# Gallicchio-Lab/openmm_agbnp_plugin

Measured on AMD Instinct MI355X. Metric: AGBNP1 force-eval-limited ns/day (1 fs step), thrombin 1dwc, independent replicas, higher is better.
Workload: dtype f64

## Files before the change

### openmm_agbnp_plugin_amd/csrc/agbnp_common.h

```cpp
#pragma once
#include <cfloat>
#include <cmath>
#include <cstddef>
#include <cstdint>

#ifdef __HIPCC__
#define AGBNP_HD __host__ __device__ __attribute__((always_inline))
#else
#define AGBNP_HD
#endif

namespace agbnp {

constexpr double kKFC = (2.2269859253f);
constexpr double kMinGvol = FLT_MIN;
constexpr int kMaxOrder = 8;
constexpr double kVolMinA = (0.01f * (0.001f));
constexpr double kVolMinB = (0.1f * (0.001f));
constexpr double kRadiusIncrement = (0.5f * (0.1f));
constexpr double kHBRadius = (1.4 * (0.1f));
constexpr double kSolventRadius = (1.0 * (0.1f));
constexpr double kI4MaxA = 2.0;
constexpr int kI4Nodes = 16;
constexpr int kLutStride = kI4Nodes + 1;
constexpr long kRadiusPrecision = 10000;
constexpr double kPi = 3.14159265358979323846;

constexpr double kToKjMol = 4.184 * 332.0 / 10.0;
constexpr double kDielFactor = kToKjMol * (-0.5) * (1. / 1.0 - 1. / 80.0);

struct SubtreeHeader {
  int nnodes;
  int natoms;
  int nroots;
  int npairs;
  int partners[8];
};



constexpr int kMaxItems = 8;
constexpr int kRowStride = 16;
AGBNP_HD constexpr size_t slot_row_item(size_t slot, size_t k) { return (size_t)kRowStride * slot + k; }
AGBNP_HD constexpr size_t slot_row_count(size_t slot) { return (size_t)kRowStride * slot + kMaxItems; }

constexpr int kWorkItemPartShift = 24, kWorkItemPartsShift = 26;
AGBNP_HD constexpr int make_work_item(int root, int part, int parts) {
  return root | (part << kWorkItemPartShift) | ((parts - 1) << kWorkItemPartsShift);
}
AGBNP_HD constexpr int work_item_root(int e) { return e & ((1 << kWorkItemPartShift) - 1); }
AGBNP_HD constexpr int work_item_part(int e) { return (e >> kWorkItemPartShift) & 3; }
AGBNP_HD constexpr int work_item_parts(int e) { return ((e >> kWorkItemPartsShift) & 3) + 1; }

constexpr int kTileBlocksMax = 4095;
constexpr int kTileStripFlag = 1 << 24;
AGBNP_HD constexpr int make_tile_item(int I, int J, int flag = 0) { return I | (J << 12) | flag; }
AGBNP_HD constexpr int tile_I(int item) { return item & 0xfff; }
AGBNP_HD constexpr int tile_J(int item) { return (item >> 12) & 0xfff; }

constexpr int kRowEntryTypeShift = 24;
AGBNP_HD constexpr unsigned make_row_entry(unsigned index, unsigned type) { return index | (type << kRowEntryTypeShift); }
AGBNP_HD constexpr unsigned row_entry_index(unsigned e) { return e & ((1u << kRowEntryTypeShift) - 1); }
AGBNP_HD constexpr unsigned row_entry_type(unsigned e) { return e >> kRowEntryTypeShift; }
constexpr int kRowItemSliceShift = 24;
AGBNP_HD constexpr unsigned make_row_item(unsigned list, unsigned slice) { return list | (slice << kRowItemSliceShift); }
AGBNP_HD constexpr unsigned row_item_list(unsigned it) { return it & ((1u << kRowItemSliceShift) - 1); }
AGBNP_HD constexpr unsigned row_item_slice(unsigned it) { return it >> kRowItemSliceShift; }

enum PackingWord {
  kPackForestsNext = 1,
  kPackForestsNow = 2,
  kPackState = 3,
};
enum PackStateWord {
  kPsLevel = 0,
  kPsAge = 1,
  kPsClean = 2,
  kPsPlans = 3,
  kPsTotalNodes = 4,
  kPsMaxNodes = 5,
  kPsEpoch = 6,
  kPsHeat = 7,
  kPsNeed = 8,
  kPsWords = 9,
  kPsReported = kPsPlans + 1
};
constexpr size_t packing_words(size_t slot_cap) { return slot_cap + kPackState + kPsWords; }

enum RowFlagWord {
  kNlStale = 0,
// ... 55 lines not shown
```

### openmm_agbnp_plugin_amd/csrc/engine_setup.hip

```cpp
#include "engine_context.h"

thread_local std::string g_create_error;

EngineSettings read_settings() {
  EngineSettings s;
  if (const char* v = getenv("AGBNP_HIP_FIVE_LAUNCHES")) s.five_launches = atoi(v) != 0;
  if (const char* v = getenv("AGBNP_HIP_ROWS")) s.rows = atoi(v) != 0 ? 1 : 0;
  if (const char* v = getenv("AGBNP_HIP_HEAL")) s.heal = atoi(v) != 0;
  if (const char* v = getenv("AGBNP_HIP_SPLIT_FIT")) s.split_fit = atoi(v) != 0;
  if (const char* v = getenv("AGBNP_HIP_GB_FAR")) s.gb_far = atoi(v) != 0 ? 1 : 0;
  if (const char* v = getenv("AGBNP_HIP_ROUND_PERMILLE")) s.round_permille = std::max(100, atoi(v));
  if (const char* v = getenv("AGBNP_HIP_REPLAN_EVERY")) s.replan_every = std::max(1, atoi(v));
  if (const char* v = getenv("AGBNP_HIP_ADAPTER_LAUNCH")) s.adapter_launch = atoi(v) != 0;
  if (getenv("AGBNP_HIP_NO_PINNED_STAGING")) s.pinned_staging = false;
  if (const char* v = getenv("AGBNP_HIP_SKIN")) s.skin = std::min(1.0, std::max(0.0, atof(v)));
  if (const char* v = getenv("AGBNP_HIP_ROW_MOVE")) s.row_move = std::max(atof(v), 0.0);
  if (const char* v = getenv("AGBNP_HIP_ROW_SLICE")) s.row_slice = atoi(v);
  if (const char* v = getenv("AGBNP_HIP_ROW_FILL")) s.row_fill = std::max(0.01, atof(v));
  if (const char* v = getenv("AGBNP_HIP_ROW_STRIDE")) s.row_stride = std::max(128, atoi(v));
  if (const char* v = getenv("AGBNP_HIP_MASK_SKIN")) s.mask_skin = std::min(0.5, std::max(0.0, atof(v)));
  if (const char* v = getenv("AGBNP_HIP_GROUP_LAUNCHES")) s.group_launches = atoi(v) != 0;
  return s;
}

// ... 180 lines not shown
  P.tree_atom_cap = tree_variant_atom_cap(c->variant);
  P.pack_enabled = 1;
  c->T.want_sv_large = c->diagnostics ? 1 : 0;
  apply_parity(c);
}

int mark_rows_stale(agbnp_hip_context* c) {
  const int stale = 1;
  HIP_TRY(c, hipMemcpy(c->d_nl_flag.p + kNlStale, &stale, sizeof(int), hipMemcpyHostToDevice));
  return AGBNP_HIP_OK;
}

namespace {

int allocate_rows(agbnp_hip_context* c) {
  const int n = c->n, nh = c->nh;
  PairArgs& P = c->P;
  constexpr int kRowCap = 3072;
  constexpr int kMaxTypes = 255;
  constexpr size_t kMaxTableBytes = 40 * 1024;
  constexpr int kMaxParticles = 65536;
  if (c->version != 1 || nh == 0 || n > kMaxParticles || c->cfg.rows == 0) return AGBNP_HIP_OK;
  if (c->lut.nscreened > kMaxTypes || c->lut.nscreener > kMaxTypes) return AGBNP_HIP_OK;
  if ((size_t)c->lut.nscreened * c->lut.nscreener * (kI4Nodes - 1) * 2 * sizeof(double2) > kMaxTableBytes) return AGBNP_HIP_OK;
  c->skin = c->cfg.skin;
  c->row_move = c->cfg.row_move;
  c->row_slice = c->cfg.row_slice;
  auto sorted_by_type = [&](int count, auto type_of) {
    std::vector<unsigned> v;
    for (int k = 0; k < count; k++) v.push_back(make_row_entry((unsigned)k, (unsigned)type_of(k)));
    std::stable_sort(v.begin(), v.end(), [](unsigned a, unsigned b) { return row_entry_type(a) < row_entry_type(b); });
    while (v.size() % 64 != 0) v.push_back(~0u);
    return v;
  };
  const std::vector<unsigned> hperm = sorted_by_type(nh, [&](int h) { return c->lut.type_screener[c->h2a[h]]; });
  const std::vector<unsigned> aperm = sorted_by_type(n, [&](int a) { return c->lut.type_screened[a]; });
  HIP_TRY(c, device_array(c, &P.hperm, hperm));
  HIP_TRY(c, device_array(c, &P.aperm, aperm));
  P.hperm_n = (int)hperm.size();
  P.aperm_n = (int)aperm.size();
  auto part_stride = [&](size_t candidates, int parts) { return std::max(128, std::min(64 * (int)((candidates / 64 + parts - 1) / parts), kRowCap)); };
  static_assert(kRowCap % 256 == 0, "a list is walked in slices of 256 entries");
  P.nlh_stride = part_stride(hperm.size(), kBornParts);
  P.nla_stride = part_stride(aperm.size(), kChainParts);
  {
    const double r = c->cutoff + c->skin + 0.3;
    const double most = 2.0 * 105.0 * (4.0 / 3.0) * M_PI * r * r * r / kGbParts;
    P.nlg_stride = c->method != 0 && c->cutoff > 0.0 && c->cutoff < 3.0
                       ? std::max(256, std::min(part_stride(aperm.size(), kGbParts), (int)((most + 255) / 256) * 256)) : 0;
  }
  if (c->cfg.row_stride > 0) {
    P.nlh_stride = P.nla_stride = c->cfg.row_stride;
    if (P.nlg_stride) P.nlg_stride = P.nlh_stride;
  }
  const size_t born_lists = (size_t)row_groups(n) * kBornParts, chain_lists = (size_t)row_groups(nh) * kChainParts;
  const size_t gb_lists = P.nlg_stride > 0 ? (size_t)row_groups(n) * kGbParts : 0;
  HIP_TRY(c, device_array(c, &P.nlh, born_lists * P.nlh_stride, 0));
  HIP_TRY(c, device_array(c, &P.nla, chain_lists * P.nla_stride, 0));
  HIP_TRY(c, device_array(c, &P.nlh_count, born_lists, 0));
  HIP_TRY(c, device_array(c, &P.nla_count, chain_lists, 0));
  {
    std::vector<unsigned> bs(row_groups(n), 0u), cs(row_groups(nh), 0u);
    for (int a = 0; a < n; a++) bs[a / kRowGroup] |= (unsigned)c->lut.type_screened[a] << (8 * (a % kRowGroup));
    for (int h = 0; h < nh; h++) cs[h / kRowGroup] |= (unsigned)c->lut.type_screener[c->h2a[h]] << (8 * (h % kRowGroup));
    HIP_TRY(c, device_array(c, &P.bslice, bs));
    HIP_TRY(c, device_array(c, &P.cslice, cs));
  }
  if (gb_lists > 0) {
    HIP_TRY(c, device_array(c, &P.nlg, gb_lists * P.nlg_stride, 0));
    HIP_TRY(c, device_array(c, &P.nlg_count, gb_lists, 0));
    const size_t waves = (gb_lists + 7) / 8 * 8 * (size_t)((P.nlg_stride + 255) / 256);
    HIP_TRY(c, c->d_egb_rows.alloc(waves, 0));
  }
  {
    const size_t most = std::max(std::max(born_lists * ((P.nlh_stride + 255) / 256), chain_lists * ((P.nla_stride + 255) / 256)),
                                 gb_lists * ((P.nlg_stride + 255) / 256));
    P.nl_items_cap = (int)std::min<size_t>(most + 8, 1u << 30);
    HIP_TRY(c, device_array(c, &P.nl_items, (size_t)kRowKinds * kRowBuffers * P.nl_items_cap, 0));
    HIP_TRY(c, device_array(c, &P.nl_nitems, kRowKinds * kRowBuffers, 0));
  }
  std::vector<int> flag(kNlFlagWords, 0);
  flag[kNlStale] = 1;
  flag[kNlSlice] = c->row_slice > 0 ? std::min(std::max(c->row_slice, kRowSlice), kRowSliceMax) / 64 * 64 : kRowSlice;
  HIP_TRY(c, c->d_nl_flag.upload(flag));
  P.nl_flag = c->d_nl_flag.p;
  HIP_TRY(c, device_array(c, &P.nl_ref, 3 * (size_t)n, 0xff));
  HIP_TRY(c, device_array(c, &P.bw, n, 0));
  HIP_TRY(c, device_array(c, &P.rec_h, nh));
  HIP_TRY(c, device_array(c, &P.hrow, nh));
  HIP_TRY(c, device_array(c, &P.grec, n, 0));
  HIP_TRY(c, device_array(c, &P.hrec, nh, 0));
  const int nti = c->lut.nscreened, ntj = c->lut.nscreener, ni = kI4Nodes - 1;
  const size_t tab = (size_t)nti * ntj * ni;
  const double dr = kI4MaxA / (kI4Nodes - 1);
  std::vector<double2> pw(4 * tab);
  for (int ti = 0; ti < nti; ti++)
    for (int tj = 0; tj < ntj; tj++)
      for (int k = 0; k < ni; k++) {
        const size_t o = ((size_t)ti * ntj + tj) * kI4Nodes + k;
        const double y0 = c->lut.y[o], y1 = c->lut.y[o + 1], z0 = c->lut.y2[o] * dr * dr / 6.0, z1 = c->lut.y2[o + 1] * dr * dr / 6.0;
        const double2 ca = make_double2(y0, (y1 - y0) - std::fma(2.0, z0, z1)), cb = make_double2(3.0 * z0, z1 - z0);
        const size_t by_screened = ((size_t)ti * ntj + tj) * ni + k, by_screener = ((size_t)tj * nti + ti) * ni + k;
        pw[by_screened] = ca;
        pw[tab + by_screened] = cb;
        pw[2 * tab + by_screener] = ca;
        pw[3 * tab + by_screener] = cb;
      }
  HIP_TRY(c, device_array(c, &P.pw_a, pw));
  P.pw_b = P.pw_a + tab;
  P.pwt_a = P.pw_a + 2 * tab;
  P.pwt_b = P.pw_a + 3 * tab;
  c->rows_capable = true;
  return AGBNP_HIP_OK;
}

int allocate_work(agbnp_hip_context* c) {
  const int n = c->n, nh = c->nh;
  PairArgs& P = c->P;
  TreeArgs& T = c->T;
  const size_t n3 = 3 * (size_t)n;
  const int nblk = (n + 63) / 64;
  {
    if (nblk > kTileBlocksMax) return c->fail(AGBNP_HIP_ERR_CAPACITY, "more than 262080 particles are not supported by the tile index encoding");
    std::vector<int> items;
    items.reserve((size_t)nblk * nblk / 2 + 4);
    for (int p2 = 0; 2 * p2 + 1 < nblk; p2++)
      for (int J = 2 * p2 + 2; J < nblk; J++) items.push_back(make_tile_item(2 * p2, J, kTileStripFlag));
    for (int p2 = 0; 2 * p2 + 1 < nblk; p2++) items.push_back(make_tile_item(2 * p2, 2 * p2 + 1));
    for (int I = 0; I < nblk; I++) items.push_back(make_tile_item(I, I));
    HIP_TRY(c, device_array(c, &P.gb_items, items));
// ... 336 lines not shown
```

### openmm_agbnp_plugin_amd/csrc/i4_tables.cpp

```cpp
#include "i4_tables.h"

#include <cmath>
#include <map>

#include "agbnp_common.h"

namespace agbnp {
namespace {

double q4_integral(double r, double Ri, double Rj) {
  const double two_pi = 2.0 * M_PI;
  if (r > Ri + Rj) {
    const double rp = r + Rj, rm = r - Rj;
    return two_pi * (Rj / (rp * rm) - 0.5 * log(rp / rm) / r);
  }
  const double gap = Rj - Ri;
  if (r * r > gap * gap) {
    const double rp = r + Rj, rm = r - Rj;
    const double inv_rp = 1. / rp, inv_ri = 1. / Ri;
    const double lg = 0.5 * log(rp / Ri);
    return two_pi * (-(inv_rp - inv_ri) + (0.25 * (rp * rm) * (inv_rp * inv_rp - inv_ri * inv_ri) - lg) / r);
  }
  if (Ri > Rj) return 0.0;
  const double rp = r + Rj, rm = Rj - r;
// ... 58 lines not shown
  for (int i = 0; i < n; i++) {
    type_screened[i] = idx_all[(long)(vdw_radius[i] * kRadiusPrecision)];
    if (!ishydrogen[i]) type_screener[i] = idx_heavy[(long)((vdw_radius[i] + 0.0) * kRadiusPrecision)];
  }

  const double rmin = 0.0, rmax = kI4MaxA;
  const double dr = (rmax - rmin) / (kI4Nodes - 1);
  const double xa = 0.5 * (rmax + rmin), xb = rmax;
  std::vector<double> x(kI4Nodes), yy(kI4Nodes);
  for (int k = 0; k < kI4Nodes; k++) x[k] = k * dr + rmin;
  y.assign((size_t)nscreened * nscreener * kI4Nodes, 0.0);
  y2.assign((size_t)nscreened * nscreener * kI4Nodes, 0.0);
  for (int ti = 0; ti < nscreened; ti++)
    for (int tj = 0; tj < nscreener; tj++) {
      const double Ri = radius_screened[ti];
      const double Rj = pow(1.0, 1. / 3.) * radius_screener[tj];
      for (int k = 0; k < kI4Nodes; k++) yy[k] = taper(x[k], xa, xb) * q4_integral(x[k], Ri, Rj);
      const size_t o = ((size_t)ti * nscreener + tj) * kI4Nodes;
      for (int k = 0; k < kI4Nodes; k++) y[o + k] = yy[k];
      natural_spline_y2(x, yy, &y2[o]);
    }
}

}
```

### openmm_agbnp_plugin_amd/csrc/i4_tables.h

```cpp
#pragma once
#include <vector>

namespace agbnp {

struct I4TableSet {
  int nscreened = 0;
  int nscreener = 0;
  std::vector<double> radius_screened, radius_screener;
  std::vector<int> type_screened;
  std::vector<int> type_screener;
  std::vector<double> y, y2;
  void build(const std::vector<double>& vdw_radius, const std::vector<int>& ishydrogen);
};

}
```

### openmm_agbnp_plugin_amd/csrc/pair_kernels.hip

```cpp
#include "pair_bodies.h"

namespace agbnp {

__global__ __launch_bounds__(256) void k_prep(PairArgs P, int prep_blocks) {
  if ((int)blockIdx.x >= prep_blocks) return neighbor_tile(P, blockIdx.x - prep_blocks);
  prep_atoms(P, blockIdx.x * blockDim.x + threadIdx.x, blockIdx.x == 0, false);
}

__global__ __launch_bounds__(256) void k_masks(PairArgs P, int ref_blocks) {
  if ((int)blockIdx.x >= ref_blocks) return neighbor_tile(P, blockIdx.x - ref_blocks);
  const int h = blockIdx.x * blockDim.x + threadIdx.x;
  if (h >= P.nh) return;
  const Pos3 r = heavy_position(P, h);
  P.mask_ref[3 * h] = r.x;
  P.mask_ref[3 * h + 1] = r.y;
  P.mask_ref[3 * h + 2] = r.z;
}

template <bool kBoth>
__device__ __forceinline__ void born_walk(double& sum_i, double& sum_j, const double2* __restrict__ s_lut,
                                          const double2* __restrict__ jxy, const double2* __restrict__ jzs,
                                          const double* __restrict__ jty, double xi, double yi, double zi, double si, int row,
                                          int tsr, int nsteps, int masked_step, bool vi, bool lower, int ntj, double range2) {
#pragma unroll 4
// ... 256 lines not shown
hipError_t launch_masks(const PairArgs& P, hipStream_t st, Timeline* tl) {
  AGBNP_MARK(kKPrep);
  const int ref_blocks = (std::max(P.nh, 1) + 255) / 256;
  hipLaunchKernelGGL(k_masks, dim3(ref_blocks + P.nb_tiles), dim3(256), 0, st, P, ref_blocks);
  return hipGetLastError();
}

hipError_t launch_prep(const PairArgs& P, hipStream_t st, Timeline* tl) {
  AGBNP_MARK(kKPrep);
  const int n = std::max(std::max(P.n, P.nslots), (int)kStatEvalWords);
  const int prep_blocks = (n + 255) / 256;
  hipLaunchKernelGGL(k_prep, dim3(prep_blocks + P.nb_tiles), dim3(256), 0, st, P, prep_blocks);
  return hipGetLastError();
}

PairLaunchShape pair_launch_shape(const PairArgs& P, int version) {
  PairLaunchShape s{};
  const int born_groups = (P.n + kRowGroup - 1) / kRowGroup, chain_groups = (P.nh + kRowGroup - 1) / kRowGroup;
  auto walk_blocks = [](int lists, int waves, int cap) { return (lists + waves - 1) / waves * ((cap + kRowSlice - 1) / kRowSlice); };
  s.born_walk = walk_blocks(born_groups * kBornParts, kRowWaves, P.nlh_cap);
  s.born_build = (chain_groups * kChainParts + (P.gb_rows ? born_groups * kGbParts : 0) + kRowWaves - 1) / kRowWaves;
  s.born_mask_from = s.born_walk + s.born_build;
  s.born_blocks = s.born_mask_from + P.nb_tiles;
  s.born_lds = (size_t)2 * P.nti * P.ntj * kRowIntervals * sizeof(double2);
  s.gb_tile_blocks = P.gb_items_count + 1;
  s.gb_row_blocks = 1 + walk_blocks(born_groups * kGbParts, kGbRowWaves, P.nlg_cap);
  s.chain_blocks = 2 + walk_blocks(chain_groups * kChainParts, kRowWaves, P.nla_cap);
  s.chain_lds = std::max(s.born_lds, sizeof(TileSums));
  s.role_blocks = 3;
  const int nh1 = std::max(P.nh, 1);
  const int classes_ints = std::min(2 * nh1 + 64, 12288), rounds_ints = std::min(nh1 + P.tree_slots + nh1 + nh1 / 4 + 64, 14000);
  const int role_bytes = version == 1 ? 0 : (int)kRoleScratchBytes + 4 * std::max(classes_ints, rounds_ints);
  const int force_blocks = (P.n + 255) / 256 + (version == 1 ? 0 : 2);
  s.out = {force_blocks, role_bytes, -1};
  s.out_masks = {force_blocks + P.nb_tiles, role_bytes, force_blocks};
  s.out_energy = {2 + P.nb_tiles, role_bytes, 2};
  return s;
}

hipError_t launch_pair_stages(const PairArgs& P, const PairLaunchShape& S, double* energy_out, double* components, hipStream_t st, Timeline* tl) {
  const size_t lds = (size_t)P.lut_entries * sizeof(double2);
  if (lds > 32 * 1024) {
    hipError_t e = hipFuncSetAttribute(reinterpret_cast<const void*>(k_born_tiles), hipFuncAttributeMaxDynamicSharedMemorySize, (int)lds);
    if (e != hipSuccess) return e;
    e = hipFuncSetAttribute(reinterpret_cast<const void*>(k_dborn_tiles), hipFuncAttributeMaxDynamicSharedMemorySize, (int)(lds + 3 * 64 * sizeof(double2)));
    if (e != hipSuccess) return e;
  }
// ... 94 lines not shown
```

### openmm_agbnp_plugin_amd/csrc/row_kernels.h

```cpp
#pragma once
#include <hip/hip_runtime.h>

#include "agbnp_common.h"
#include "device_math.h"
#include "pair_kernels.h"

#ifndef PAIR_STAMP
#define PAIR_STAMP(kern, idx)
#define PAIR_STAMP_WAIT(kern, idx, what)
#define PAIR_STAMP_WHERE(kern, item)
#endif
#ifndef PAIR_STAMP_HW
#define PAIR_STAMP_HW(kern)
#endif
#ifndef ROWS_LOG_COUNTS
#define ROWS_LOG_COUNTS(kern, todo, nsteps)
#endif

namespace agbnp {

__device__ __forceinline__ void hbm_add(double* p, double v) {
  __hip_atomic_fetch_add(p, v, __ATOMIC_RELAXED, __HIP_MEMORY_SCOPE_AGENT);
}

// ... 31 lines not shown
  e_atom[a] = al / bh3 + kDielFactor * q * q * r.inv_br;
  brw[a] = brw_a;
  if (add_bw) hbm_add(&bw[a], bw_alpha(r, brw_a, q));
  return brw_a;
}
template <class real>
struct GbPairTerms {
  real s1, mw, ybb, ets3;
};
__device__ __forceinline__ double gb_exp2(double y) { return exp2_nonpositive(y); }
__device__ __forceinline__ float gb_exp2(float y) { return __builtin_amdgcn_exp2f(y); }
__device__ __forceinline__ double gb_rsqrt(double u) { return rsqrt_pos(u); }
__device__ __forceinline__ float gb_rsqrt(float u) { return __builtin_amdgcn_rsqf(u); }
template <class real>
__device__ __forceinline__ GbPairTerms<real> gb_pair_terms(real d2, real bb, real c, real qq) {
  const real et = gb_exp2(d2 * c), fgb = gb_rsqrt(fma(bb, et, d2));
  GbPairTerms<real> t;
  t.s1 = qq * fgb;
  const real s3 = t.s1 * (fgb * fgb);
  t.mw = fma((real)-0.25, et, (real)1) * s3, t.ybb = fma((real)0.25, d2, bb), t.ets3 = et * s3;
  return t;
}

constexpr int kRowIntervals = kI4Nodes - 1;

__device__ __forceinline__ int uniform(int v) { return __builtin_amdgcn_readfirstlane(v); }
__device__ __forceinline__ double uniform(double v) {
  return __hiloint2double(__builtin_amdgcn_readfirstlane(__double2hiint(v)), __builtin_amdgcn_readfirstlane(__double2loint(v)));
}
template <int kCtrl>
__device__ __forceinline__ double dpp_move(double v) {
  const int lo = __builtin_amdgcn_update_dpp(0, __double2loint(v), kCtrl, 0xf, 0xf, true);
  const int hi = __builtin_amdgcn_update_dpp(0, __double2hiint(v), kCtrl, 0xf, 0xf, true);
  return __hiloint2double(hi, lo);
}
__device__ __forceinline__ double lane_xor1(double v) { return dpp_move<0xB1>(v); }
__device__ __forceinline__ double lane_xor2(double v) { return dpp_move<0x4E>(v); }
__device__ __forceinline__ double lane_xor4(double v) { return dpp_move<0x1B>(dpp_move<0x141>(v)); }
__device__ __forceinline__ double lane_xor8(double v) { return dpp_move<0x128>(v); }

enum RowKind { kBornRows = 0, kChainRows = 1, kGbRows = 2 };
struct RowAtoms {
  double x[kRowGroup], y[kRowGroup], z[kRowGroup];
  int self[kRowGroup];
  int rows;
};

// ... 55 lines not shown
  const int wgs = (items + kRowWaves - 1) / kRowWaves, rs = nl_flag[kNlSlice];
  if (wgs > row_target && wgs <= 2 * row_target && rs < kRowSliceMax) {
    nl_flag[kNlSlice] = max(rs, kRowSlice) + 64;
    nl_flag[kNlStale] = 1;
  }
}

struct RowLists {
  unsigned* list;
  int* count;
  int stride, cap, groups, parts;
};
template <int KIND>
__device__ __forceinline__ RowLists row_lists(const PairArgs& P) {
  RowLists L;
  L.list = KIND == kBornRows ? P.nlh : KIND == kChainRows ? P.nla : P.nlg;
  L.count = KIND == kBornRows ? P.nlh_count : KIND == kChainRows ? P.nla_count : P.nlg_count;
  L.stride = KIND == kBornRows ? P.nlh_stride : KIND == kChainRows ? P.nla_stride : P.nlg_stride;
  L.cap = KIND == kBornRows ? P.nlh_cap : KIND == kChainRows ? P.nla_cap : P.nlg_cap;
  L.groups = ((KIND == kChainRows ? P.nh : P.n) + kRowGroup - 1) / kRowGroup;
  L.parts = KIND == kBornRows ? kBornParts : KIND == kChainRows ? kChainParts : kGbParts;
  return L;
}
template <int KIND>
__device__ __forceinline__ void append_items(const PairArgs& P, int sub, int entries, bool at_least_one) {
  const int rs = row_slice_length(P);
  const int nsl = max((entries + rs - 1) / rs, at_least_one ? 1 : 0);
  if (nsl == 0) return;
  const int buf = (P.nl_flag[kNlBuilds] + 1) & 1;
  const int base = atomicAdd(&P.nl_nitems[kRowBuffers * KIND + buf], nsl);
  unsigned* items = P.nl_items + (size_t)(kRowBuffers * KIND + buf) * P.nl_items_cap;
  for (int sl = 0; sl < nsl && base + sl < P.nl_items_cap; sl++) items[base + sl] = make_row_item((unsigned)sub, (unsigned)sl);
}

template <int KIND>
__device__ __forceinline__ void build_list(const PairArgs& P, int sub, int lane, int stale, int* estatus) {
  const RowLists L = row_lists<KIND>(P);
  if (sub >= L.groups * L.parts) return;
  if (!stale) {
    if (lane == 0 && L.count[sub] > L.cap) estatus[kStatRowOverflow] = 1;
    return;
  }
  const int g = sub / L.parts, part = sub - g * L.parts;
  const RowAtoms A = row_atoms<KIND>(P, g);
  const int cnt = row_build(A, P.aperm, P.aperm_n, part, L.parts, static_cast<const double4*>(P.aposq), KIND == kGbRows ? P.nlg_build2 : P.nl_build2,
                            L.list + (size_t)sub * L.stride, L.stride, lane);
  if (lane == 0) {
    L.count[sub] = cnt;
    if (cnt > L.cap) estatus[kStatRowOverflow] = 1;
    append_items<KIND>(P, sub, min(cnt, L.cap), KIND == kGbRows && part == 0);
  }
}

template <int KIND>
constexpr int kRowStamp = KIND == kChainRows ? 2 : KIND == kGbRows ? 1 : 0;
__device__ __forceinline__ int rebuild_born_list(const PairArgs& P, const RowLists& L, const RowAtoms& A, int sub, int group, int part, int slice, int first, int lane,
                                                 int* estatus, unsigned& e1, unsigned& e2) {
  const unsigned* list = P.nlh + (size_t)sub * L.stride;
  int count = row_build(A, P.hperm, P.hperm_n, part, L.parts, static_cast<const double4*>(P.rec_h), P.nl_build2, P.nlh + (size_t)sub * L.stride, L.stride, lane);
  if (lane == 0 && slice == 0) {
    P.nlh_count[sub] = count;
    if (count > L.cap) estatus[kStatRowOverflow] = 1;
    append_items<kBornRows>(P, sub, min(count, L.cap), false);
  }
  if (slice == 0 && part == 0 && lane < A.rows) {
    const int a = kRowGroup * group + lane;
    const double4 pa = static_cast<const double4*>(P.aposq)[a];
    P.nl_ref[3 * a] = pa.x, P.nl_ref[3 * a + 1] = pa.y, P.nl_ref[3 * a + 2] = pa.z;
  }
  __builtin_amdgcn_fence(__ATOMIC_SEQ_CST, "workgroup");
  e1 = list[min(first + lane, L.stride - 1)], e2 = list[min(first + 64 + lane, L.stride - 1)];
  return min(count, L.stride);
}

template <int KIND, int WAVES, bool SINGLE = false, bool PARITY = false>
__device__ __forceinline__ void rows_workgroup(const PairArgs& P, int blk, double2* s_dyn, int* s_busy_word) {
  static_assert(!SINGLE || KIND != kGbRows, "the GB rows choose their precision at run time (P.single)");
  constexpr int R = kRowGroup;
  static_assert(R == 4, "the butterfly below folds 16 sums");
  int& s_busy = *s_busy_word;
  const int lane = threadIdx.x & 63, wave = __builtin_amdgcn_readfirstlane(threadIdx.x >> 6);
  const RowLists L = row_lists<KIND>(P);
  const int NP = L.parts, stride = L.stride;
  const int nlists = L.groups * NP, lists_pad = (nlists + WAVES - 1) / WAVES * WAVES;
  const int stale = P.nl_flag[kNlStale];
  const int epoch_now = PARITY ? P.epoch[0] : 0;
  const int rs = row_slice_length(P);
  const int walk_blocks = lists_pad / WAVES * ((L.cap + kRowSlice - 1) / kRowSlice);
  auto flag_row_overflow = [&]() { P.estatus[(PARITY ? kStatBlockStride * (epoch_now & 1) : 0) + kStatRowOverflow] = 1; };
  if (KIND == kBornRows && blk >= walk_blocks) {
    const int sub = (blk - walk_blocks) * WAVES + wave;
    const int chain_lists = row_lists<kChainRows>(P).groups * kChainParts;
    if (sub < chain_lists)
      build_list<kChainRows>(P, sub, lane, stale, P.estatus + (PARITY ? kStatBlockStride * (epoch_now & 1) : 0));
    else if (P.gb_rows)
      build_list<kGbRows>(P, sub - chain_lists, lane, stale, P.estatus + (PARITY ? kStatBlockStride * (epoch_now & 1) : 0));
    return;
  }
  PAIR_STAMP(kRowStamp<KIND>, 0);
  const int item = blk * WAVES + wave;
  const bool compact = !(KIND == kBornRows && stale);
  int slice, li;
  bool active;
  if (compact) {
    const int buf = (P.nl_flag[kNlBuilds] + (stale ? 1 : 0)) & 1;
    const int nitems = min(P.nl_nitems[kRowBuffers * KIND + buf], P.nl_items_cap);
    if (blk * WAVES >= nitems) {
      if (KIND == kGbRows && lane == 0 && item < P.egb_parts) P.egb_part[item] = 0.0;
      return;
    }
    PAIR_STAMP_HW(kRowStamp<KIND>);
    PAIR_STAMP(kRowStamp<KIND>, 10);
    active = item < nitems;
    const unsigned it = (P.nl_items + (size_t)(kRowBuffers * KIND + buf) * P.nl_items_cap)[active ? item : 0];
    PAIR_STAMP_WAIT(kRowStamp<KIND>, 11, "vmcnt(0)");
    li = (int)row_item_list(it);
    slice = (int)row_item_slice(it);
  } else {
    slice = item / lists_pad, li = item - slice * lists_pad;
    active = li < nlists;
  }
  const int sub = active ? li : 0;
  const int group = sub / NP, part = sub - group * NP;
  const unsigned* list = L.list + (size_t)sub * stride;
  const int first = rs * slice;
  const int listed_raw = L.count[sub];
  const int listed = min(listed_raw, stride);
  unsigned e1 = list[min(first + lane, stride - 1)], e2 = list[min(first + 64 + lane, stride - 1)];
  const unsigned types = KIND == kGbRows ? 0u : (KIND == kChainRows ? P.cslice : P.bslice)[group];
  const RowAtoms A = row_atoms<KIND>(P, group);
  double row_rv[R], row_bp[R], row_q[R];
  if (KIND == kGbRows) {
#pragma unroll
    for (int r = 0; r < R; r++) {
      const int a = min(R * group + r, P.n - 1);
      row_rv[r] = P.inv_rvdw[a], row_bp[r] = P.born_part[a], row_q[r] = static_cast<const double4*>(P.aposq)[a].w;
    }
  }
  const int ne = (KIND == kChainRows ? P.nti : P.ntj) * kRowIntervals;
  const int tab = P.nti * P.ntj * kRowIntervals;
  double2* const s_tab = s_dyn;
  constexpr int kWg = 64 * WAVES;
  const double2* __restrict__ gtab = KIND == kChainRows ? P.pwt_a : P.pw_a;
  const int tx = threadIdx.x;
  const bool mine = active && ((KIND == kBornRows && stale) || first < listed || (KIND == kGbRows && slice == 0 && part == 0));
  if (KIND == kGbRows && lane == 0 && !mine && item < P.egb_parts) P.egb_part[item] = 0.0;
  if (!compact) {
    if (threadIdx.x == 0) s_busy = 0;
    __syncthreads();
    if (mine && lane == 0) s_busy = 1;
    __syncthreads();
    if (!s_busy) return;
  }
  float4* const s_tab4 = reinterpret_cast<float4*>(s_dyn);
  double2 tv0, tv1, tv2, tv3;
  if (KIND != kGbRows && !SINGLE) tv0 = gtab[min(tx, 2 * tab - 1)], tv1 = gtab[min(kWg + tx, 2 * tab - 1)], tv2 = gtab[min(2 * kWg + tx, 2 * tab - 1)];
  if (KIND != kGbRows && SINGLE)
    tv0 = gtab[min(tx, tab - 1)], tv1 = gtab[tab + min(tx, tab - 1)], tv2 = gtab[min(kWg + tx, tab - 1)], tv3 = gtab[tab + min(kWg + tx, tab - 1)];
  PAIR_STAMP_WAIT(kRowStamp<KIND>, 7, "vmcnt(0) lgkmcnt(0)");
  if (KIND != kGbRows && !SINGLE) {
    if (tx < 2 * tab) s_tab[tx] = tv0;
    if (kWg + tx < 2 * tab) s_tab[kWg + tx] = tv1;
    if (2 * kWg + tx < 2 * tab) s_tab[2 * kWg + tx] = tv2;
    for (int base = 3 * kWg; base < 2 * tab; base += kWg)
      if (base + tx < 2 * tab) s_tab[base + tx] = gtab[base + tx];
  }
  if (KIND != kGbRows && SINGLE) {
    if (tx < tab) s_tab4[tx] = make_float4((float)tv0.x, (float)tv0.y, (float)tv1.x, (float)tv1.y);
    if (kWg + tx < tab) s_tab4[kWg + tx] = make_float4((float)tv2.x, (float)tv2.y, (float)tv3.x, (float)tv3.y);
    for (int base = 2 * kWg; base < tab; base += kWg)
      if (base + tx < tab) {
        const double2 a = gtab[base + tx], b = gtab[tab + base + tx];
        s_tab4[base + tx] = make_float4((float)a.x, (float)a.y, (float)b.x, (float)b.y);
      }
  }
  int slice_at[R];
#pragma unroll
  for (int r = 0; r < R; r++) slice_at[r] = uniform((int)((types >> (8 * r)) & 0xffu) * ne);
  int count = listed;
  if (KIND == kBornRows && stale && active) {
    count = rebuild_born_list(P, L, A, sub, group, part, slice, first, lane, P.estatus + (PARITY ? kStatBlockStride * (epoch_now & 1) : 0), e1, e2);
  }
  if (KIND == kBornRows && active && slice == 0 && lane == 0 && !stale && listed_raw > L.cap) flag_row_overflow();
  const int todo = active ? max(0, min(count - first, rs)) : 0;
  const int nsteps = (todo + 63) >> 6;
  double acc[4 * R];
#pragma unroll
  for (int q = 0; q < 4 * R; q++) acc[q] = 0.0;
  constexpr double kPerNode = (kI4Nodes - 1) / kI4MaxA;
  double esum = 0.0;
  double beta_r[R];
  if (KIND != kGbRows) {
    const double4* __restrict__ rec = KIND == kChainRows ? static_cast<const double4*>(P.aposq) : static_cast<const double4*>(P.rec_h);
    const double* __restrict__ wsrc = KIND == kChainRows ? static_cast<const double*>(P.bw)
                                                          : static_cast<const double*>(P.sv_vdw) + (PARITY ? (size_t)(epoch_now & 1) * P.table_doubles : 0);
    double4 r1 = rec[row_entry_index(e1)];
    double w1 = wsrc[row_entry_index(e1)];
    __syncthreads();
    PAIR_STAMP(kRowStamp<KIND>, 8);
    PAIR_STAMP_WAIT(kRowStamp<KIND>, 1, "vmcnt(0)");
    ROWS_LOG_COUNTS(kRowStamp<KIND>, todo, nsteps);
    if (SINGLE) {
      float ox[R], oy[R], oz[R], accf[4 * R];
#pragma unroll
      for (int r = 0; r < R; r++) ox[r] = (float)(A.x[r] - A.x[0]), oy[r] = (float)(A.y[r] - A.y[0]), oz[r] = (float)(A.z[r] - A.z[0]);
#pragma unroll
      for (int q = 0; q < 4 * R; q++) accf[q] = 0.0f;
      const float per_node = (float)kPerNode, range2f = (float)P.range2;
      for (int k = 0; k < nsteps; k++) {
        const unsigned e = e1;
        const double4 rb = r1;
        const double wb = w1;
        e1 = e2;
        r1 = rec[row_entry_index(e1)];
        w1 = wsrc[row_entry_index(e1)];
        e2 = list[min(first + 64 * (k + 2) + lane, stride - 1)];
        const int b = (int)row_entry_index(e);
        const int tent = (int)row_entry_type(e) * kRowIntervals;
        const float w = (float)((KIND == kChainRows ? wb : wb * rb.w) * kPerNode);
        const float cut2 = 64 * k + lane < todo ? range2f : -1.0f;
        const float nx = (float)(rb.x - A.x[0]), ny = (float)(rb.y - A.y[0]), nz = (float)(rb.z - A.z[0]);
#pragma unroll
        for (int r = 0; r < R; r++) {
          const float dx = nx - ox[r], dy = ny - oy[r], dz = nz - oz[r];
          const float d2 = fmaf(dz, dz, fmaf(dy, dy, dx * dx));
          if (d2 < cut2 && b != A.self[r]) {
            const float rinv = __builtin_amdgcn_rsqf(d2);
            const float u = fminf((d2 * rinv) * per_node, (float)kRowIntervals - 1e-3f);
            const int ent = slice_at[r] + tent + (int)u;
            const float t = u - (float)(int)u;
            const float4 c = s_tab4[ent];
            const float b2 = fmaf(c.w, t, c.z), b1 = fmaf(b2, t, c.y);
            const float val = fmaf(b1, t, c.x), der = fmaf(fmaf(c.w, t, b2), t, b1);
            accf[4 * r] = fmaf(w, val, accf[4 * r]);
            const float g = w * der * rinv;
            accf[4 * r + 1] = fmaf(dx, g, accf[4 * r + 1]);
            accf[4 * r + 2] = fmaf(dy, g, accf[4 * r + 2]);
            accf[4 * r + 3] = fmaf(dz, g, accf[4 * r + 3]);
          }
        }
      }
#pragma unroll
      for (int q = 0; q < 4 * R; q++) acc[q] = (double)accf[q];
    } else
    for (int k = 0; k < nsteps; k++) {
      const unsigned e = e1;
      const double4 rb = r1;
      const double wb = w1;
      e1 = e2;
      r1 = rec[row_entry_index(e1)];
      w1 = wsrc[row_entry_index(e1)];
      e2 = list[min(first + 64 * (k + 2) + lane, stride - 1)];
      const int b = (int)row_entry_index(e);
      const int tent = (int)row_entry_type(e) * kRowIntervals;
      const double w = (KIND == kChainRows ? wb : wb * rb.w) * kPerNode;
      const double range2 = 64 * k + lane < todo ? P.range2 : -1.0;
#pragma unroll
      for (int r = 0; r < R; r++) {
        const double dx = rb.x - A.x[r], dy = rb.y - A.y[r], dz = rb.z - A.z[r];
        const double d2 = fma(dz, dz, fma(dy, dy, dx * dx));
        if (d2 < range2 && b != A.self[r]) {
          const double rinv = rsqrt_pos(d2);
          const double u = fmin((d2 * rinv) * kPerNode, kRowIntervals - 0x1p-49);
          const int ent = slice_at[r] + tent + (int)u;
          const double t = __builtin_amdgcn_fract(u);
          const double2 ca = s_tab[ent], cb = s_tab[ent + tab];
          const double b2 = fma(cb.y, t, cb.x), b1 = fma(b2, t, ca.y);
          const double val = fma(b1, t, ca.x), der = fma(fma(cb.y, t, b2), t, b1);
          acc[4 * r] = fma(w, val, acc[4 * r]);
          const double g = w * der * rinv;
          acc[4 * r + 1] = fma(dx, g, acc[4 * r + 1]);
          acc[4 * r + 2] = fma(dy, g, acc[4 * r + 2]);
          acc[4 * r + 3] = fma(dz, g, acc[4 * r + 3]);
        }
      }
    }
  } else {
    const double4* __restrict__ rec = static_cast<const double4*>(P.aposq);
    double qa[R], ba[R], ca_[R];
    BornRadius bra[R];
#pragma unroll
    for (int r = 0; r < R; r++) {
      bra[r] = born_radius(row_rv[r], row_bp[r]);
      qa[r] = uniform(r < A.rows ? row_q[r] : 0.0);
      ba[r] = uniform(bra[r].br);
      ca_[r] = uniform((-0.25 * 1.4426950408889634074) * bra[r].inv_br);
      beta_r[r] = bw_beta(bra[r]);
    }
    if (active && slice == 0 && part == 0 && lane < A.rows) {
      BornRadius br = bra[0];
      double qv = row_q[0];
#pragma unroll
      for (int r = 1; r < R; r++) {
        if (lane == r) br = bra[r], qv = row_q[r];
      }
      publish_atom(R * group + lane, br, qv, P.alpha, P.born, P.born_fp, P.e_atom, P.brw, P.bw, true);
    }
    double4 r1 = rec[row_entry_index(e1)];
    double p1 = P.born_part[row_entry_index(e1)], v1 = P.inv_rvdw[row_entry_index(e1)];
    PAIR_STAMP(kRowStamp<KIND>, 8);
    PAIR_STAMP_WAIT(kRowStamp<KIND>, 1, "vmcnt(0)");
    ROWS_LOG_COUNTS(kRowStamp<KIND>, todo, nsteps);
    if (P.single) {
      float ox[R], oy[R], oz[R], qf[R], bf[R], cf[R], accf[4 * R];
#pragma unroll
      for (int r = 0; r < R; r++) {
        ox[r] = (float)(A.x[r] - A.x[0]), oy[r] = (float)(A.y[r] - A.y[0]), oz[r] = (float)(A.z[r] - A.z[0]);
        qf[r] = (float)qa[r], bf[r] = (float)ba[r], cf[r] = (float)ca_[r];
      }
#pragma unroll
      for (int q = 0; q < 4 * R; q++) accf[q] = 0.0f;
      float esumf = 0.0f;
// ... 97 lines not shown
```

Measured before the change: 885.9.

## Pad I4 spline tables with an end entry and balance row-slice spans

Each type pair's spline table gets one extra entry holding the constant value and slope at the end of the last interval. With that entry in place, the per-pair fmin clamp on the interval coordinate can be dropped in both the f32 and f64 row loops. Row work items now carry an explicit start and step count, so a list's 64-entry steps are spread evenly across its slices instead of leaving a short final slice. The costs are a slightly larger LDS table with an index remap during the table load, and tighter bit-field limits on the work-item encoding, which are checked at allocation.

```diff
diff --git a/openmm_agbnp_plugin_amd/csrc/agbnp_common.h b/openmm_agbnp_plugin_amd/csrc/agbnp_common.h
--- a/openmm_agbnp_plugin_amd/csrc/agbnp_common.h
+++ b/openmm_agbnp_plugin_amd/csrc/agbnp_common.h
@@ -23,6 +23,7 @@
 constexpr double kI4MaxA = 2.0;
 constexpr int kI4Nodes = 16;
 constexpr int kLutStride = kI4Nodes + 1;
+constexpr int kRowTabEntries = kI4Nodes, kRowTabStride = kRowTabEntries + 1;
 constexpr long kRadiusPrecision = 10000;
 constexpr double kPi = 3.14159265358979323846;
 
@@ -62,10 +63,29 @@
 AGBNP_HD constexpr unsigned make_row_entry(unsigned index, unsigned type) { return index | (type << kRowEntryTypeShift); }
 AGBNP_HD constexpr unsigned row_entry_index(unsigned e) { return e & ((1u << kRowEntryTypeShift) - 1); }
 AGBNP_HD constexpr unsigned row_entry_type(unsigned e) { return e >> kRowEntryTypeShift; }
-constexpr int kRowItemSliceShift = 24;
-AGBNP_HD constexpr unsigned make_row_item(unsigned list, unsigned slice) { return list | (slice << kRowItemSliceShift); }
-AGBNP_HD constexpr unsigned row_item_list(unsigned it) { return it & ((1u << kRowItemSliceShift) - 1); }
-AGBNP_HD constexpr unsigned row_item_slice(unsigned it) { return it >> kRowItemSliceShift; }
+struct RowSpan {
+  int first, steps, todo;
+};
+AGBNP_HD constexpr int row_slices(int count, int cap, int rs) { return ((count < cap ? count : cap) + rs - 1) / rs; }
+AGBNP_HD constexpr RowSpan row_slice_span_of(int walked, int nsl, int q, int s) {
+  if (s < 0 || s >= nsl) return RowSpan{walked, 0, 0};
+  const int steps = (walked + 63) >> 6, longer_from = nsl - (steps - q * nsl);
+  const int mine = q + (s >= longer_from ? 1 : 0), before = s * q + (s > longer_from ? s - longer_from : 0);
+  const int left = walked - 64 * before;
+  return RowSpan{64 * before, mine, left < 64 * mine ? left : 64 * mine};
+}
+AGBNP_HD constexpr RowSpan row_slice_span(int count, int cap, int rs, int s) {
+  const int walked = count < cap ? count : cap, nsl = (walked + rs - 1) / rs;
+  return row_slice_span_of(walked, nsl, nsl > 0 ? ((walked + 63) >> 6) / nsl : 0, s);
+}
+constexpr int kRowItemFirstShift = 17, kRowItemStepsShift = 25;
+constexpr int kRowItemListsMax = 1 << kRowItemFirstShift, kRowItemEntriesMax = 64 << (kRowItemStepsShift - kRowItemFirstShift);
+AGBNP_HD constexpr unsigned make_row_item(unsigned list, unsigned first, unsigned steps) {
+  return list | ((first / 64) << kRowItemFirstShift) | (steps << kRowItemStepsShift);
+}
+AGBNP_HD constexpr unsigned row_item_list(unsigned it) { return it & ((1u << kRowItemFirstShift) - 1); }
+AGBNP_HD constexpr unsigned row_item_first(unsigned it) { return 64 * ((it >> kRowItemFirstShift) & ((1u << (kRowItemStepsShift - kRowItemFirstShift)) - 1)); }
+AGBNP_HD constexpr unsigned row_item_steps(unsigned it) { return (it >> kRowItemStepsShift) & 15u; }
 
 enum PackingWord {
   kPackForestsNext = 1,
diff --git a/openmm_agbnp_plugin_amd/csrc/engine_setup.hip b/openmm_agbnp_plugin_amd/csrc/engine_setup.hip
--- a/openmm_agbnp_plugin_amd/csrc/engine_setup.hip
+++ b/openmm_agbnp_plugin_amd/csrc/engine_setup.hip
@@ -226,7 +226,7 @@
   constexpr int kMaxParticles = 65536;
   if (c->version != 1 || nh == 0 || n > kMaxParticles || c->cfg.rows == 0) return AGBNP_HIP_OK;
   if (c->lut.nscreened > kMaxTypes || c->lut.nscreener > kMaxTypes) return AGBNP_HIP_OK;
-  if ((size_t)c->lut.nscreened * c->lut.nscreener * (kI4Nodes - 1) * 2 * sizeof(double2) > kMaxTableBytes) return AGBNP_HIP_OK;
+  if ((size_t)c->lut.nscreened * c->lut.nscreener * kRowTabStride * 2 * sizeof(double2) > kMaxTableBytes) return AGBNP_HIP_OK;
   c->skin = c->cfg.skin;
   c->row_move = c->cfg.row_move;
   c->row_slice = c->cfg.row_slice;
@@ -259,6 +259,10 @@
   }
   const size_t born_lists = (size_t)row_groups(n) * kBornParts, chain_lists = (size_t)row_groups(nh) * kChainParts;
   const size_t gb_lists = P.nlg_stride > 0 ? (size_t)row_groups(n) * kGbParts : 0;
+  static_assert((size_t)(kMaxParticles / kRowGroup) * kChainParts <= (size_t)kRowItemListsMax && kRowCap <= kRowItemEntriesMax &&
+                    kRowSliceMax / 64 < 16,
+                "the fields of a row launch's work item");
+  if (std::max(std::max(P.nlh_stride, P.nla_stride), P.nlg_stride) > kRowItemEntriesMax) return AGBNP_HIP_OK;
   HIP_TRY(c, device_array(c, &P.nlh, born_lists * P.nlh_stride, 0));
   HIP_TRY(c, device_array(c, &P.nla, chain_lists * P.nla_stride, 0));
   HIP_TRY(c, device_array(c, &P.nlh_count, born_lists, 0));
@@ -294,22 +298,10 @@
   HIP_TRY(c, device_array(c, &P.hrow, nh));
   HIP_TRY(c, device_array(c, &P.grec, n, 0));
   HIP_TRY(c, device_array(c, &P.hrec, nh, 0));
-  const int nti = c->lut.nscreened, ntj = c->lut.nscreener, ni = kI4Nodes - 1;
-  const size_t tab = (size_t)nti * ntj * ni;
-  const double dr = kI4MaxA / (kI4Nodes - 1);
+  const size_t tab = (size_t)c->lut.nscreened * c->lut.nscreener * kRowTabEntries;
+  const std::vector<double> coefficients = c->lut.power_form();
   std::vector<double2> pw(4 * tab);
-  for (int ti = 0; ti < nti; ti++)
-    for (int tj = 0; tj < ntj; tj++)
-      for (int k = 0; k < ni; k++) {
-        const size_t o = ((size_t)ti * ntj + tj) * kI4Nodes + k;
-        const double y0 = c->lut.y[o], y1 = c->lut.y[o + 1], z0 = c->lut.y2[o] * dr * dr / 6.0, z1 = c->lut.y2[o + 1] * dr * dr / 6.0;
-        const double2 ca = make_double2(y0, (y1 - y0) - std::fma(2.0, z0, z1)), cb = make_double2(3.0 * z0, z1 - z0);
-        const size_t by_screened = ((size_t)ti * ntj + tj) * ni + k, by_screener = ((size_t)tj * nti + ti) * ni + k;
-        pw[by_screened] = ca;
-        pw[tab + by_screened] = cb;
-        pw[2 * tab + by_screener] = ca;
-        pw[3 * tab + by_screener] = cb;
-      }
+  for (size_t k = 0; k < 4 * tab; k++) pw[k] = make_double2(coefficients[2 * k], coefficients[2 * k + 1]);
   HIP_TRY(c, device_array(c, &P.pw_a, pw));
   P.pw_b = P.pw_a + tab;
   P.pwt_a = P.pw_a + 2 * tab;
diff --git a/openmm_agbnp_plugin_amd/csrc/i4_tables.cpp b/openmm_agbnp_plugin_amd/csrc/i4_tables.cpp
--- a/openmm_agbnp_plugin_amd/csrc/i4_tables.cpp
+++ b/openmm_agbnp_plugin_amd/csrc/i4_tables.cpp
@@ -104,4 +104,32 @@
     }
 }
 
+std::vector<double> I4TableSet::power_form() const {
+  const int nti = nscreened, ntj = nscreener, ni = kI4Nodes - 1;
+  const size_t tab = (size_t)nti * ntj * kRowTabEntries;
+  const double dr = kI4MaxA / (kI4Nodes - 1);
+  std::vector<double> pw(2 * 4 * tab, 0.0);
+  for (int ti = 0; ti < nti; ti++)
+    for (int tj = 0; tj < ntj; tj++) {
+      const size_t by_screened = ((size_t)ti * ntj + tj) * kRowTabEntries, by_screener = ((size_t)tj * nti + ti) * kRowTabEntries;
+      auto put = [&](int k, double c0, double c1, double c2, double c3) {
+        for (const size_t at : {by_screened + k, 2 * tab + by_screener + k}) {
+          pw[2 * at] = c0, pw[2 * at + 1] = c1;
+          pw[2 * (tab + at)] = c2, pw[2 * (tab + at) + 1] = c3;
+        }
+      };
+      double c0 = 0.0, c1 = 0.0, c2 = 0.0, c3 = 0.0;
+      for (int k = 0; k < ni; k++) {
+        const size_t o = ((size_t)ti * ntj + tj) * kI4Nodes + k;
+        const double y0 = y[o], y1 = y[o + 1], z0 = y2[o] * dr * dr / 6.0, z1 = y2[o + 1] * dr * dr / 6.0;
+        c0 = y0, c1 = (y1 - y0) - std::fma(2.0, z0, z1), c2 = 3.0 * z0, c3 = z1 - z0;
+        put(k, c0, c1, c2, c3);
+      }
+      static_assert(kRowTabEntries == kI4Nodes, "the intervals of a type pair and the end of the last one");
+      const double b2 = c3 + c2, b1 = b2 + c1;
+      put(ni, b1 + c0, (c3 + b2) + b1, 0.0, 0.0);
+    }
+  return pw;
 }
+
+}
diff --git a/openmm_agbnp_plugin_amd/csrc/i4_tables.h b/openmm_agbnp_plugin_amd/csrc/i4_tables.h
--- a/openmm_agbnp_plugin_amd/csrc/i4_tables.h
+++ b/openmm_agbnp_plugin_amd/csrc/i4_tables.h
@@ -11,6 +11,7 @@
   std::vector<int> type_screener;
   std::vector<double> y, y2;
   void build(const std::vector<double>& vdw_radius, const std::vector<int>& ishydrogen);
+  std::vector<double> power_form() const;
 };
 
 }
diff --git a/openmm_agbnp_plugin_amd/csrc/pair_kernels.hip b/openmm_agbnp_plugin_amd/csrc/pair_kernels.hip
--- a/openmm_agbnp_plugin_amd/csrc/pair_kernels.hip
+++ b/openmm_agbnp_plugin_amd/csrc/pair_kernels.hip
@@ -302,7 +302,7 @@
   s.born_build = (chain_groups * kChainParts + (P.gb_rows ? born_groups * kGbParts : 0) + kRowWaves - 1) / kRowWaves;
   s.born_mask_from = s.born_walk + s.born_build;
   s.born_blocks = s.born_mask_from + P.nb_tiles;
-  s.born_lds = (size_t)2 * P.nti * P.ntj * kRowIntervals * sizeof(double2);
+  s.born_lds = (size_t)2 * P.nti * P.ntj * kRowTabStride * sizeof(double2);
   s.gb_tile_blocks = P.gb_items_count + 1;
   s.gb_row_blocks = 1 + walk_blocks(born_groups * kGbParts, kGbRowWaves, P.nlg_cap);
   s.chain_blocks = 2 + walk_blocks(chain_groups * kChainParts, kRowWaves, P.nla_cap);
diff --git a/openmm_agbnp_plugin_amd/csrc/row_kernels.h b/openmm_agbnp_plugin_amd/csrc/row_kernels.h
--- a/openmm_agbnp_plugin_amd/csrc/row_kernels.h
+++ b/openmm_agbnp_plugin_amd/csrc/row_kernels.h
@@ -77,7 +77,7 @@
   return t;
 }
 
-constexpr int kRowIntervals = kI4Nodes - 1;
+__device__ __forceinline__ int row_tab_lds(int g) { return g + g / kRowTabEntries * (kRowTabStride - kRowTabEntries); }
 
 __device__ __forceinline__ int uniform(int v) { return __builtin_amdgcn_readfirstlane(v); }
 __device__ __forceinline__ double uniform(double v) {
@@ -179,15 +179,21 @@
   L.parts = KIND == kBornRows ? kBornParts : KIND == kChainRows ? kChainParts : kGbParts;
   return L;
 }
+__device__ __forceinline__ int small_quotient(int a, int b) { return (int)(((float)a + 0.5f) * __builtin_amdgcn_rcpf((float)b)); }
 template <int KIND>
 __device__ __forceinline__ void append_items(const PairArgs& P, int sub, int entries, bool at_least_one) {
   const int rs = row_slice_length(P);
-  const int nsl = max((entries + rs - 1) / rs, at_least_one ? 1 : 0);
+  const int slices = small_quotient(entries + rs - 1, rs);
+  const int q = small_quotient((entries + 63) >> 6, max(slices, 1));
+  const int nsl = max(slices, at_least_one ? 1 : 0);
   if (nsl == 0) return;
   const int buf = (P.nl_flag[kNlBuilds] + 1) & 1;
   const int base = atomicAdd(&P.nl_nitems[kRowBuffers * KIND + buf], nsl);
   unsigned* items = P.nl_items + (size_t)(kRowBuffers * KIND + buf) * P.nl_items_cap;
-  for (int sl = 0; sl < nsl && base + sl < P.nl_items_cap; sl++) items[base + sl] = make_row_item((unsigned)sub, (unsigned)sl);
+  for (int sl = 0; sl < nsl && base + sl < P.nl_items_cap; sl++) {
+    const RowSpan span = row_slice_span_of(entries, slices, q, sl);
+    items[base + sl] = make_row_item((unsigned)sub, (unsigned)span.first, (unsigned)span.steps);
+  }
 }
 
 template <int KIND>
@@ -211,16 +217,16 @@
 
 template <int KIND>
 constexpr int kRowStamp = KIND == kChainRows ? 2 : KIND == kGbRows ? 1 : 0;
-__device__ __forceinline__ int rebuild_born_list(const PairArgs& P, const RowLists& L, const RowAtoms& A, int sub, int group, int part, int slice, int first, int lane,
+__device__ __forceinline__ int rebuild_born_list(const PairArgs& P, const RowLists& L, const RowAtoms& A, int sub, int group, int part, int first, int lane,
                                                  int* estatus, unsigned& e1, unsigned& e2) {
   const unsigned* list = P.nlh + (size_t)sub * L.stride;
   int count = row_build(A, P.hperm, P.hperm_n, part, L.parts, static_cast<const double4*>(P.rec_h), P.nl_build2, P.nlh + (size_t)sub * L.stride, L.stride, lane);
-  if (lane == 0 && slice == 0) {
+  if (lane == 0 && first == 0) {
     P.nlh_count[sub] = count;
     if (count > L.cap) estatus[kStatRowOverflow] = 1;
     append_items<kBornRows>(P, sub, min(count, L.cap), false);
   }
-  if (slice == 0 && part == 0 && lane < A.rows) {
+  if (first == 0 && part == 0 && lane < A.rows) {
     const int a = kRowGroup * group + lane;
     const double4 pa = static_cast<const double4*>(P.aposq)[a];
     P.nl_ref[3 * a] = pa.x, P.nl_ref[3 * a + 1] = pa.y, P.nl_ref[3 * a + 2] = pa.z;
@@ -257,7 +263,7 @@
   PAIR_STAMP(kRowStamp<KIND>, 0);
   const int item = blk * WAVES + wave;
   const bool compact = !(KIND == kBornRows && stale);
-  int slice, li;
+  int li, first, span;
   bool active;
   if (compact) {
     const int buf = (P.nl_flag[kNlBuilds] + (stale ? 1 : 0)) & 1;
@@ -272,15 +278,16 @@
     const unsigned it = (P.nl_items + (size_t)(kRowBuffers * KIND + buf) * P.nl_items_cap)[active ? item : 0];
     PAIR_STAMP_WAIT(kRowStamp<KIND>, 11, "vmcnt(0)");
     li = (int)row_item_list(it);
-    slice = (int)row_item_slice(it);
+    first = (int)row_item_first(it), span = 64 * (int)row_item_steps(it);
   } else {
-    slice = item / lists_pad, li = item - slice * lists_pad;
+    const int slice = item / lists_pad;
+    li = item - slice * lists_pad;
+    first = rs * slice, span = rs;
     active = li < nlists;
   }
   const int sub = active ? li : 0;
   const int group = sub / NP, part = sub - group * NP;
   const unsigned* list = L.list + (size_t)sub * stride;
-  const int first = rs * slice;
   const int listed_raw = L.count[sub];
   const int listed = min(listed_raw, stride);
   unsigned e1 = list[min(first + lane, stride - 1)], e2 = list[min(first + 64 + lane, stride - 1)];
@@ -294,13 +301,14 @@
       row_rv[r] = P.inv_rvdw[a], row_bp[r] = P.born_part[a], row_q[r] = static_cast<const double4*>(P.aposq)[a].w;
     }
   }
-  const int ne = (KIND == kChainRows ? P.nti : P.ntj) * kRowIntervals;
-  const int tab = P.nti * P.ntj * kRowIntervals;
+  const int ne = (KIND == kChainRows ? P.nti : P.ntj) * kRowTabStride;
+  const int tab = P.nti * P.ntj * kRowTabEntries;
+  const int ltab = P.nti * P.ntj * kRowTabStride;
   double2* const s_tab = s_dyn;
   constexpr int kWg = 64 * WAVES;
   const double2* __restrict__ gtab = KIND == kChainRows ? P.pwt_a : P.pw_a;
   const int tx = threadIdx.x;
-  const bool mine = active && ((KIND == kBornRows && stale) || first < listed || (KIND == kGbRows && slice == 0 && part == 0));
+  const bool mine = active && ((KIND == kBornRows && stale) || first < listed || (KIND == kGbRows && first == 0 && part == 0));
   if (KIND == kGbRows && lane == 0 && !mine && item < P.egb_parts) P.egb_part[item] = 0.0;
   if (!compact) {
     if (threadIdx.x == 0) s_busy = 0;
@@ -316,19 +324,19 @@
     tv0 = gtab[min(tx, tab - 1)], tv1 = gtab[tab + min(tx, tab - 1)], tv2 = gtab[min(kWg + tx, tab - 1)], tv3 = gtab[tab + min(kWg + tx, tab - 1)];
   PAIR_STAMP_WAIT(kRowStamp<KIND>, 7, "vmcnt(0) lgkmcnt(0)");
   if (KIND != kGbRows && !SINGLE) {
-    if (tx < 2 * tab) s_tab[tx] = tv0;
-    if (kWg + tx < 2 * tab) s_tab[kWg + tx] = tv1;
-    if (2 * kWg + tx < 2 * tab) s_tab[2 * kWg + tx] = tv2;
+    if (tx < 2 * tab) s_tab[row_tab_lds(tx)] = tv0;
+    if (kWg + tx < 2 * tab) s_tab[row_tab_lds(kWg + tx)] = tv1;
+    if (2 * kWg + tx < 2 * tab) s_tab[row_tab_lds(2 * kWg + tx)] = tv2;
     for (int base = 3 * kWg; base < 2 * tab; base += kWg)
-      if (base + tx < 2 * tab) s_tab[base + tx] = gtab[base + tx];
+      if (base + tx < 2 * tab) s_tab[row_tab_lds(base + tx)] = gtab[base + tx];
   }
   if (KIND != kGbRows && SINGLE) {
-    if (tx < tab) s_tab4[tx] = make_float4((float)tv0.x, (float)tv0.y, (float)tv1.x, (float)tv1.y);
-    if (kWg + tx < tab) s_tab4[kWg + tx] = make_float4((float)tv2.x, (float)tv2.y, (float)tv3.x, (float)tv3.y);
+    if (tx < tab) s_tab4[row_tab_lds(tx)] = make_float4((float)tv0.x, (float)tv0.y, (float)tv1.x, (float)tv1.y);
+    if (kWg + tx < tab) s_tab4[row_tab_lds(kWg + tx)] = make_float4((float)tv2.x, (float)tv2.y, (float)tv3.x, (float)tv3.y);
     for (int base = 2 * kWg; base < tab; base += kWg)
       if (base + tx < tab) {
         const double2 a = gtab[base + tx], b = gtab[tab + base + tx];
-        s_tab4[base + tx] = make_float4((float)a.x, (float)a.y, (float)b.x, (float)b.y);
+        s_tab4[row_tab_lds(base + tx)] = make_float4((float)a.x, (float)a.y, (float)b.x, (float)b.y);
       }
   }
   int slice_at[R];
@@ -336,10 +344,10 @@
   for (int r = 0; r < R; r++) slice_at[r] = uniform((int)((types >> (8 * r)) & 0xffu) * ne);
   int count = listed;
   if (KIND == kBornRows && stale && active) {
-    count = rebuild_born_list(P, L, A, sub, group, part, slice, first, lane, P.estatus + (PARITY ? kStatBlockStride * (epoch_now & 1) : 0), e1, e2);
-  }
-  if (KIND == kBornRows && active && slice == 0 && lane == 0 && !stale && listed_raw > L.cap) flag_row_overflow();
-  const int todo = active ? max(0, min(count - first, rs)) : 0;
+    count = rebuild_born_list(P, L, A, sub, group, part, first, lane, P.estatus + (PARITY ? kStatBlockStride * (epoch_now & 1) : 0), e1, e2);
+  }
+  if (KIND == kBornRows && active && first == 0 && lane == 0 && !stale && listed_raw > L.cap) flag_row_overflow();
+  const int todo = active ? max(0, min((compact ? min(count, L.cap) : count) - first, span)) : 0;
   const int nsteps = (todo + 63) >> 6;
   double acc[4 * R];
 #pragma unroll
@@ -373,7 +381,7 @@
         w1 = wsrc[row_entry_index(e1)];
         e2 = list[min(first + 64 * (k + 2) + lane, stride - 1)];
         const int b = (int)row_entry_index(e);
-        const int tent = (int)row_entry_type(e) * kRowIntervals;
+        const int tent = (int)row_entry_type(e) * kRowTabStride;
         const float w = (float)((KIND == kChainRows ? wb : wb * rb.w) * kPerNode);
         const float cut2 = 64 * k + lane < todo ? range2f : -1.0f;
         const float nx = (float)(rb.x - A.x[0]), ny = (float)(rb.y - A.y[0]), nz = (float)(rb.z - A.z[0]);
@@ -383,7 +391,7 @@
           const float d2 = fmaf(dz, dz, fmaf(dy, dy, dx * dx));
           if (d2 < cut2 && b != A.self[r]) {
             const float rinv = __builtin_amdgcn_rsqf(d2);
-            const float u = fminf((d2 * rinv) * per_node, (float)kRowIntervals - 1e-3f);
+            const float u = (d2 * rinv) * per_node;
             const int ent = slice_at[r] + tent + (int)u;
             const float t = u - (float)(int)u;
             const float4 c = s_tab4[ent];
@@ -409,7 +417,7 @@
       w1 = wsrc[row_entry_index(e1)];
       e2 = list[min(first + 64 * (k + 2) + lane, stride - 1)];
       const int b = (int)row_entry_index(e);
-      const int tent = (int)row_entry_type(e) * kRowIntervals;
+      const int tent = (int)row_entry_type(e) * kRowTabStride;
       const double w = (KIND == kChainRows ? wb : wb * rb.w) * kPerNode;
       const double range2 = 64 * k + lane < todo ? P.range2 : -1.0;
 #pragma unroll
@@ -418,10 +426,10 @@
         const double d2 = fma(dz, dz, fma(dy, dy, dx * dx));
         if (d2 < range2 && b != A.self[r]) {
           const double rinv = rsqrt_pos(d2);
-          const double u = fmin((d2 * rinv) * kPerNode, kRowIntervals - 0x1p-49);
+          const double u = (d2 * rinv) * kPerNode;
           const int ent = slice_at[r] + tent + (int)u;
           const double t = __builtin_amdgcn_fract(u);
-          const double2 ca = s_tab[ent], cb = s_tab[ent + tab];
+          const double2 ca = s_tab[ent], cb = s_tab[ent + ltab];
           const double b2 = fma(cb.y, t, cb.x), b1 = fma(b2, t, ca.y);
           const double val = fma(b1, t, ca.x), der = fma(fma(cb.y, t, b2), t, b1);
           acc[4 * r] = fma(w, val, acc[4 * r]);
@@ -444,7 +452,7 @@
       ca_[r] = uniform((-0.25 * 1.4426950408889634074) * bra[r].inv_br);
       beta_r[r] = bw_beta(bra[r]);
     }
-    if (active && slice == 0 && part == 0 && lane < A.rows) {
+    if (active && first == 0 && part == 0 && lane < A.rows) {
       BornRadius br = bra[0];
       double qv = row_q[0];
 #pragma unroll
```

New measurement: 891.0, median of 6. About the same (+0.6%).
